# fnzhan/EMLight

Measured on AMD Instinct MI355X. Metric: training images/sec (regression step: DenseNet-BC fwd + Sinkhorn loss + bwd + Adam), higher is better.
Workload: dtype f32; 1 GPU; RegressionNetwork train step, BASELINE configs[1]; per_gpu_batch=64, global_batch=64, anchors=128, parallelism=single

## Files before the change

emlight_amd/RegressionNetwork/dense_engine_bwd.py:

```python
import ctypes
import os

import torch

from .. import _lib
from .._knobs import knob_choice, knob_flag


def _r16(v):
    return (v + 15) // 16 * 16


class _BwdBuffers:
    def gf12(self, r):
        if self.GF12[r] is None:
            self.GF12[r] = self._gf12_new()
        return self.GF12[r]

    def __init__(self, enc, ws, dev):
        f32 = dict(dtype=torch.float32, device=dev)
        self.G = [torch.zeros(blk["P"], blk["ld"], **f32) for blk in ws.blocks]
        self.GF = torch.zeros(ws.F.shape[0], ws.F.shape[1], **f32)
        maxP = ws.blocks[0]["P"]
        self.DZ = torch.empty(2, maxP, 48, **f32)
        self.ring = max(1, int(os.environ.get("EML_WGRAD_RING", 4))) if enc.overlap_wgrad(dev) else 1
        self.GF12 = [None] * self.ring
        self._gf12_new = lambda: torch.empty(maxP, 12, **f32)
        self.N12 = torch.empty(maxP, 12, **f32)
        self.TOP = torch.empty(2 * maxP * 12, **f32)
        kp, ko, g = enc.kp_max, max(enc.ko_max, 48), enc.grid_max
        self.Wd = [[torch.empty(lay["Kp"] * 48, **f32) for lay in blk["layers"]] for blk in ws.blocks]
        self.WdT = [torch.empty(blk["trans"]["Kp"] * blk["trans"]["Ko"], **f32) for blk in ws.blocks]
        self.permutes = None
        self.coef = torch.zeros(8, max(kp, ko), **f32)
        self.part2 = torch.zeros(2, g * kp * 2, dtype=torch.float64, device=dev)
        self.partW = torch.empty(g * max(kp * 48, 2 * 27 * 256, 4 * 1024), **f32)
        i32 = dict(dtype=torch.int32, device=dev)
        self.cond = [[torch.zeros(lay["Kp"], **i32) for lay in blk["layers"]] for blk in ws.blocks]
        self.condT = [torch.zeros(blk["trans"]["Kp"], **i32) for blk in ws.blocks]
        self.any_ill = torch.zeros(1, **i32)
        self.dg_grid = 128
        self.dg_scratch = torch.empty(self.dg_grid * kp, dtype=torch.float64, device=dev)
        self.side = None
        if enc.overlap_wgrad(dev):
            self.side = torch.cuda.Stream(device=dev)
            self.partW3 = [torch.empty(g * 2 * 27 * 256, **f32) for _ in range(self.ring)]
            self.ev_ready = [torch.cuda.Event() for _ in range(self.ring)]
            self.ev_done = [None] * self.ring


def run_backward(enc, ws, x, gpooled, need_x=False, need_params=None):
    if getattr(ws, "bwd", None) is None:
        ws.bwd = _BwdBuffers(enc, ws, x.device)
    L, p, st = _lib.lib(), _lib.ptr, _lib.current_stream()
    m = enc.model
    f = m.features
    if not m.training:
        raise NotImplementedError("HIP DenseNet backward is implemented for train-mode BatchNorm "
# ... 23 lines not shown
        for l_, lay_ in enumerate(blk_["layers"]):
            items.append((getattr(mod_, "denselayer%d" % (l_ + 1)).conv1.weight, bw.Wd[bi_][l_], 2, 48, lay_["Cin"],
                          lay_["Kp"], 48))
        tr_ = blk_["trans"]
        items.append((getattr(f, "transition%d" % (bi_ + 1)).conv.weight, bw.WdT[bi_], 2, tr_["Cout"], blk_["Ctot"],
                      tr_["Kp"], tr_["Ko"]))
    bw.permutes.launch(L, st, items)
    params = enc.param_list()
    if need_params is None:
        need_params = [True] * len(params)
    from .._dist import grad_slot
    grads = {}
    for q, need in zip(params, need_params):
        slot = grad_slot(q) if need else None
        grads[id(q)] = slot if slot is not None else torch.empty_like(q)
    gr = lambda q: p(grads[id(q)])
    coefs = [tuple(bw.coef[3 * k + i] for i in range(3)) for k in range(2)]
    cA, cB, cC = coefs[0]
    sB, sC = bw.coef[6], bw.coef[7]

    direct = knob_choice("EML_DGAMMA_DIRECT", "always", ("always", "never")) != "never"
    c3_fold = knob_flag("EML_C3_FOLD", True)
    c3_gf = knob_flag("EML_C3_GF", False)
    bw.any_ill.zero_()

    def dgamma_direct(blk, X_ld, Pin, Hin, Win, pool, DY, ld_dy, Zr, ld_z, co, Cout, conv, Cin, scale1, shift1, cond, bn):
        if not direct:
            return
        a, b, c = co if co is not None else (None, None, None)
        _lib.check(L.eml_dense_bn_dgamma_direct_f32(
            p(blk["X"]), X_ld, Pin, Hin, Win, pool, p(DY), ld_dy, p(Zr), ld_z, p(a), p(b), p(c), Cout, p(conv.weight), Cin,
            p(scale1), p(shift1), p(blk["mean"]), p(blk["istd"]), p(cond), p(bw.dg_scratch), gr(bn.weight), bw.dg_grid, st),
            "eml_dense_bn_dgamma_direct_f32")

    def finalize(R, pstride, count, bn, mean, istd, C, Cpad, coef=0, s_acc=None, src=None, c_lo=0, c_hi=None, conv=None,
                 cond=None):
        a, b, c = coefs[coef] if coef is not None else (None, None, None)
        wargs = (p(bn.bias), p(conv.weight), gr(conv.weight), conv.weight.shape[0]) if conv is not None else (None, None, None, 0)
        _lib.check(L.eml_dense_bn_bwd_finalize_f32(
            p(part if src is None else src), R, pstride, float(count), p(bn.weight), p(mean), p(istd), C, Cpad, 1,
            gr(bn.weight), gr(bn.bias), p(a), p(b), p(c),
            p(sB) if s_acc is not None else None, p(sC) if s_acc is not None else None, int(bool(s_acc)),
            c_lo, Cpad if c_hi is None else c_hi, *wargs, p(cond), p(bw.any_ill) if cond is not None else None, st),
            "eml_dense_bn_bwd_finalize_f32")

    def parr(tensors):
# ... 52 lines not shown
                                          p(part), G3d, p(blk["X"]), ld, cin, p(sB), p(sC), p(bw.gf12(r)) if c3_gf else None,
                                          p(lay["scale2"]), p(lay["shift2"]), p(bw.partW), gr(Lm.conv2.weight), *drop, st), fn)
            else:
                fn = "eml_dense_conv3x3_bwd_data_drop_f32" if drop else "eml_dense_conv3x3_bwd_data_f32"
                _lib.check(getattr(L, fn)(*gsrc, p(Lm.conv2.weight), p(z), p(lay["zmean"]), p(lay["zistd"]), p(dz), B, Hb, Wb,
                                          p(part), G3d, p(blk["X"]), ld, cin, p(sB), p(sC), p(bw.gf12(r)), *drop, st), fn)
            if fold:
                pass
            elif bw.side is None:
                _lib.check(L.eml_dense_conv3x3_bwd_weight_f32(p(bw.gf12(r)), 12, 0, p(z), p(lay["scale2"]),
                                                              p(lay["shift2"]), B, Hb, Wb, p(bw.partW),
                                                              gr(Lm.conv2.weight), G3, st),
                           "eml_dense_conv3x3_bwd_weight_f32")
            else:
                bw.ev_ready[r].record(main)
                bw.side.wait_event(bw.ev_ready[r])
                _lib.check(L.eml_dense_conv3x3_bwd_weight_f32(p(bw.gf12(r)), 12, 0, p(z), p(lay["scale2"]),
                                                              p(lay["shift2"]), B, Hb, Wb, p(bw.partW3[r]),
                                                              gr(Lm.conv2.weight), G3s, st_side),
                           "eml_dense_conv3x3_bwd_weight_f32")
                if bw.ev_done[r] is None:
                    bw.ev_done[r] = torch.cuda.Event()
                bw.ev_done[r].record(bw.side)
            finalize(G3d, 96, P, Lm.norm2, lay["zmean"], lay["zistd"], 48, 48, coef=slot)
            a, b, c = coefs[slot]
            _lib.check(L.eml_dense_conv1x1_bwd_weight_f32(
                p(blk["X"]), ld, P, Hb, Wb, 0, kp, cin, p(lay["scale1"]), p(lay["shift1"]), p(dz), 48, p(z), 48,
                p(a), p(b), p(c), 48, p(bw.partW), gr(Lm.conv1.weight), Gw, p(dz),
                *((p(Lm.conv1.weight), narrow_lo, *((p(top2[0]), 12) if top else (p(Gbuf), ld)), p(bw.N12),
                   p(bw.part2[slot])) if narrow_lo is not None
                  else (None, 0, None, 0, None, None)), st), "eml_dense_conv1x1_bwd_weight_f32")
            return Lm

        def dgrad(layers, slots, k_lo, k_hi, top=False):
            lays = [blk["layers"][l] for l in layers]
            if top:
                _lib.check(L.eml_dense_conv1x1_bwd_data_multi_top_f32(
                    parr([bw.DZ[s_] for s_ in slots]), parr([bw.Wd[bi][l_] for l_ in layers]),
                    parr([y["scale1"] for y in lays]), parr([y["shift1"] for y in lays]),
                    parr([bw.part2[s_] for s_ in slots]), (ctypes.c_int * len(layers))(*[y["Kp"] for y in lays]),
                    P, k_hi, p(Gbuf), ld, Gd, parr([y["mask"] for y in lays]), p(top2), st),
                    "eml_dense_conv1x1_bwd_data_multi_top_f32")
                return
            _lib.check(L.eml_dense_conv1x1_bwd_data_multi_f32(
                len(layers), parr([bw.DZ[s_] for s_ in slots]), None, None, None, None,
                parr([bw.Wd[bi][l_] for l_ in layers]),
                parr([y["scale1"] for y in lays]), parr([y["shift1"] for y in lays]),
                parr([bw.part2[s_] for s_ in slots]), (ctypes.c_int * len(layers))(*[y["Kp"] for y in lays]),
                None, ld, None, None, P, k_lo, k_hi, p(Gbuf), ld, Gd,
                parr([y["mask"] for y in lays]), st),
                "eml_dense_conv1x1_bwd_data_multi_f32")

        def bn1_finalize(l, Lm, slot, c_lo, c_hi, rows=None):
            lay = blk["layers"][l]
            finalize(Gd if rows is None else rows, 2 * lay["Kp"], P, Lm.norm1, blk["mean"], blk["istd"], lay["Cin"], lay["Kp"], coef=None,
                     s_acc=True, src=bw.part2[slot], c_lo=c_lo, c_hi=c_hi, conv=Lm.conv1, cond=bw.cond[bi][l])

        def bn1_direct(l, Lm, slot):
            lay = blk["layers"][l]
            dgamma_direct(blk, ld, P, Hb, Wb, 0, bw.DZ[slot], 48, None, 0, None, 48, Lm.conv1, lay["Cin"], lay["scale1"],
                          lay["shift1"], bw.cond[bi][l], Lm.norm1)

        l = len(blk["layers"]) - 1
        have_top = False
        while l >= 0:
            if l >= 1:
                la, lb = l, l - 1
                cin_a, cin_b = blk["layers"][la]["Cin"], blk["layers"][lb]["Cin"]
                Lma = conv2_backward(la, 0, narrow_lo=cin_b, top=have_top)
                bn1_finalize(la, Lma, 0, cin_b, cin_a, rows=Gw)
                Lmb = conv2_backward(lb, 1, n12=True)
                to_top = (lb >= 2 and blk["layers"][la]["mask"] is not None and bw.side is None
                          and cin_b >= 24 and cin_b % 4 == 0)
                dgrad([la, lb], [0, 1], 0, cin_b, top=to_top)
                have_top = to_top
                bn1_finalize(la, Lma, 0, 0, cin_b)
                bn1_finalize(lb, Lmb, 1, 0, blk["layers"][lb]["Kp"])
                bn1_direct(la, Lma, 0)
                bn1_direct(lb, Lmb, 1)
                l -= 2
            else:
                Lm0 = conv2_backward(l, 0)
                dgrad([l], [0], 0, blk["layers"][l]["Cin"])
                bn1_finalize(l, Lm0, 0, 0, blk["layers"][l]["Kp"])
                bn1_direct(l, Lm0, 0)
                l -= 1
        c0b = blk["C0"]
        norm0_fused = bi == 0 and knob_flag("EML_NORM0_FUSED", True) and c0b % 4 == 0 and c0b <= 32
        if not norm0_fused:
            materialize(Gbuf, blk, 0, c0b)
        dY, ld_dy = Gbuf, ld
    b0 = ws.blocks[0]
    c0 = enc.c_init
    if norm0_fused:
        _lib.check(L.eml_dense_norm0_bwd_stats_f32(p(dY), ld_dy, p(ws.Y0), c0, p(ws.scale0), p(ws.shift0), p(sB), p(sC), c0,
                                                   b0["P"], p(ws.mean0), p(ws.istd0), p(part), Gb, st),
                   "eml_dense_norm0_bwd_stats_f32")
    else:
        _lib.check(L.eml_dense_bn_bwd_stats_f32(p(dY), ld_dy, p(ws.Y0), c0, p(b0["X"]), b0["ld"], 1, c0, b0["P"],
                                                p(ws.mean0), p(ws.istd0), p(part), Gb, st), "eml_dense_bn_bwd_stats_f32")
    finalize(Gb, 2 * c0, b0["P"], f.norm0, ws.mean0, ws.istd0, c0, _r16(c0), coef=0)
    if norm0_fused:
# ... 18 lines not shown
```

emlight_amd/_knobs.py:

```python
import os
import sys

_seen = {}


def _note(name, value, default):
    if value != default:
        print("emlight_amd: A/B knob %s=%r (default %r)" % (name, value, default), file=sys.stderr)


def knob_int(name, default, lo=None, hi=None):
    raw = os.environ.get(name)
    if ("int", name, raw) not in _seen:
        val = default
        if raw is not None:
            try:
                val = int(raw)
                if (lo is not None and val < lo) or (hi is not None and val > hi):
                    raise ValueError("out of range")
            except ValueError:
                print("emlight_amd: ignoring %s=%r (want an integer%s); using %r"
                      % (name, raw, "" if lo is None else " >= %d" % lo, default), file=sys.stderr)
                val = default
        _note(name, val, default)
# ... 8 lines not shown
        if raw is not None:
            if raw in ("0", "1"):
                val = raw == "1"
            else:
                print("emlight_amd: ignoring %s=%r (want 0 or 1); using %d" % (name, raw, int(default)), file=sys.stderr)
        _note(name, val, bool(default))
        _seen[("flag", name, raw)] = val
    return _seen[("flag", name, raw)]


def knob_choice(name, default, choices):
    raw = os.environ.get(name)
    if ("choice", name, raw) not in _seen:
        val = default
        if raw is not None:
            if raw in choices:
                val = raw
            else:
                print("emlight_amd: ignoring %s=%r (want one of %s); using %r" % (name, raw, "/".join(choices), default),
                      file=sys.stderr)
        _note(name, val, default)
        _seen[("choice", name, raw)] = val
    return _seen[("choice", name, raw)]
```

emlight_amd/_lib.py:

```python
import ctypes
import os
import threading

_HERE = os.path.dirname(os.path.abspath(__file__))
LIB_PATH = os.environ.get("EML_LIB_PATH") or os.path.join(_HERE, "libemlight_hip.so")

_f32p = ctypes.c_void_p
_i32p = ctypes.c_void_p
_f64p = ctypes.c_void_p
_stream = ctypes.c_void_p
_int = ctypes.c_int
_u64 = ctypes.c_ulonglong

ABI_VERSION = 31

SIGNATURES = {
    "eml_abi_version": (_int, []),
    "eml_last_error": (ctypes.c_char_p, []),
    "eml_sg_rasterise_f32": (_int, [_f32p, _f32p, _f32p, _f32p, _int, _int, _int, _int, _stream]),
    "eml_sg_rasterise_ex_f32": (_int, [_f32p, _f32p, _f32p, _f32p, _int, _int, _int, _int, _int, ctypes.c_void_p, _stream]),
    "eml_sg_rasterise_bwd_colors_f32": (_int, [_f32p, _f32p, _f32p, _f32p, _int, _int, _int, _int, _stream]),
    "eml_emd_anchor_cost_f32": (_int, [_f32p, _f32p, _int, _stream]),
    "eml_sinkhorn_schedule_f32": (_int, [_f32p, _f32p, ctypes.c_long, ctypes.c_double, ctypes.c_double, _int,
                                         ctypes.c_double, _f32p, _f32p, _i32p, _f32p, _stream]),
# ... 202 lines not shown
    "eml_sphere_render_bwd_work_floats": (ctypes.c_size_t, [_int, _int, _int, _int]),
    "eml_sphere_render_bwd_f32": (_int, [_f32p, _int, _int, _int, _int, ctypes.c_double, _int, ctypes.c_double, _i32p, _i32p,
                                         _f32p, _f32p, _f32p, _stream]),
    "eml_sphere_mirror_taps_f32": (_int, [_int, _int, _int, ctypes.c_double, _i32p, _f32p, _stream]),
    "eml_gm_anchor_cost_f32": (_int, [ctypes.c_void_p, _int, _int, _int, _f32p, _f32p, _stream]),
    "eml_sinkhorn_fwd_cost_f32": (_int, [_f32p, _f32p, _f32p, _f32p, _f32p, _f32p, ctypes.c_double, ctypes.c_double, _int,
                                         ctypes.c_double, _f32p, _f32p, _i32p, _f32p, _f32p, _f32p, _f32p, _f32p, _int, _int,
                                         _int, _int, ctypes.c_double, _f32p, ctypes.c_long, _stream]),
    "eml_sphere_max_pool_fwd_f32": (_int, [_f32p, _i32p, _f32p, _f32p, ctypes.c_void_p, _int, _int, _int, _int, _stream]),
    "eml_sphere_max_pool_bwd_f32": (_int, [_f32p, ctypes.c_void_p, _i32p, _i32p, _f32p, _f32p, _int, _int, _int, _int, _stream]),
    "eml_sphere_conv_small_dbias_f32": (_int, [_f32p, _f32p, ctypes.c_float, _f32p, _f32p, _int, _int, _int, _int, _stream]),
    "eml_env_prefilter_work_floats": (ctypes.c_size_t, [_int, _int, _int, _int, _int]),
    "eml_env_prefilter_f32": (_int, [_f32p, _int, _int, _int, _int, _int, ctypes.c_void_p, _f32p, _f32p, _stream]),
    "eml_gbuffer_shade_f32": (_int, [_f32p, _int, _f32p, _int, ctypes.c_long, _f32p, _int, ctypes.c_long, _f32p, _f32p, _f32p,
                                     _f32p, _f32p, _int, _int, _int, ctypes.c_double, ctypes.c_double, _f32p, _f32p, _f32p,
                                     ctypes.c_double, _f32p, _stream]),
    "eml_env_prefilter_bwd_work_floats": (ctypes.c_size_t, [_int, _int, _int, _int, _int]),
    "eml_env_prefilter_bwd_f32": (_int, [_f32p, _int, _int, _int, _int, _int, ctypes.c_void_p, _f32p, _f32p, _stream]),
    "eml_gbuffer_shade_bwd_work_floats": (ctypes.c_size_t, [_int, _int, _int, _int, _int, _int, _int, _int, _int]),
    "eml_gbuffer_shade_bwd_f32": (_int, [_f32p, _f32p, _int, _f32p, _int, ctypes.c_long, _f32p, _int, ctypes.c_long, _f32p,
                                         _f32p, _f32p, _f32p, _f32p, _int, _int, _int, ctypes.c_double, ctypes.c_double,
                                         _f32p, _f32p, ctypes.c_double, _f32p, _f32p, _f32p, _f32p, _f32p, _f32p, _f32p,
                                         _f32p, _stream]),
}

_lock = threading.Lock()
_lib = None


class EmlightHipError(RuntimeError):
    pass


def lib():
    global _lib
    if _lib is not None:
        return _lib
    with _lock:
        if _lib is not None:
            return _lib
        if not os.path.exists(LIB_PATH):
            raise EmlightHipError(
                "libemlight_hip.so not found at %s -- build it with "
                "`python -c 'import __graft_entry__ as g; g.build()'` or `make -C emlight_amd/csrc`. "
                "There is no CPU fallback." % LIB_PATH)
        handle = ctypes.CDLL(LIB_PATH)
# ... 52 lines not shown
```

emlight_amd/csrc/dense_bwd.hip:

```cpp
#include "eml_common.h"
#include "eml_dropout.h"

#include <cstdint>
#include <cstdlib>
#include <type_traits>

namespace {

using eml::f32x4;
using eml::f4c;
using eml::mfma16;
using eml::shfl_xor_d;

constexpr int kTH = 8, kTW = 32, kHH = kTH + 2, kHW = kTW + 2;

constexpr int kPSG = 14;
constexpr int kBD = 512;
constexpr int kGRows = 2;
constexpr int kGPass = kHH / kGRows;

template <bool FUSE, bool WIDE, bool DROP = false>
__global__ __launch_bounds__(kBD, 2) void conv3x3_bwd_data_kernel(
    const float* __restrict__ G, int ldg, int c0, const float* __restrict__ W2, const float* __restrict__ Z,
    const float* __restrict__ zmean, const float* __restrict__ zistd, float* __restrict__ DZ, int B, int H, int W,
// ... 1543 lines not shown
    }
  }
  __syncthreads();
  for (int e = tid; e < Kp * 2; e += 256)
    partials[(size_t)blockIdx.x * Kp * 2 + e] =
        (sacc[e] + sacc[(size_t)Kp * 2 + e]) + (sacc[(size_t)2 * Kp * 2 + e] + sacc[(size_t)3 * Kp * 2 + e]);
}

struct BwdLayer {
  const float* DZ;
  const float* Zr;
  const float* cA;
  const float* cB;
  const float* cC;
  const float* Wd;
  const float* scale1;
  const float* shift1;
  double* partials;
  int Kp;
};

template <int NL, int MT , bool RAW = false ,
          bool MASKED = false, bool TOP = false>
__global__ __launch_bounds__(256, 2) void conv1x1_bwd_data_multi_kernel(BwdLayer L0, BwdLayer L1,
                                                                        const float* __restrict__ X, int ldx,
                                                                        const float* __restrict__ mean,
                                                                        const float* __restrict__ istd, int P,
                                                                        int k_lo, int k_hi, float* __restrict__ Gd,
                                                                        int ldg, int KpMax,
                                                                        const unsigned long long* __restrict__ M0,
                                                                        const unsigned long long* __restrict__ M1,
                                                                        float* __restrict__ Top) {
  extern __shared__ __attribute__((aligned(16))) float smem[];
  double* sacc = reinterpret_cast<double*>(smem);
  float* vec_l = reinterpret_cast<float*>(sacc + (size_t)NL * 4 * KpMax * 2);
  const int tid = threadIdx.x, lane = tid & 63, wave = tid >> 6;
  const int r = lane & 15, kk = lane >> 4;
  const BwdLayer Ls[2] = {L0, L1};
  for (int e = tid; e < NL * 4 * KpMax * 2; e += 256) sacc[e] = 0.0;
  for (int e = tid; e < KpMax; e += 256) {
    vec_l[e] = MASKED ? 0.f : mean[e];
    vec_l[KpMax + e] = MASKED ? 0.f : istd[e];
#pragma unroll
    for (int j = 0; j < NL; ++j) {
      vec_l[(2 + 2 * j) * KpMax + e] = e < Ls[j].Kp ? Ls[j].scale1[e] : 0.f;
      vec_l[(3 + 2 * j) * KpMax + e] = e < Ls[j].Kp ? Ls[j].shift1[e] : 0.f;
    }
  }
  __syncthreads();
  constexpr int TP = 64 * MT;
  const int ntiles = (P + TP - 1) / TP;
  const int nt_lo = k_lo >> 4, nt_hi = (k_hi + 15) >> 4;
  constexpr int NCH = 2;

  float4 wq[2][3][NCH];
  auto load_w = [&](int j, int nt0, float4 (&dst)[3][NCH]) {
    const int nnt = Ls[j].Kp >> 4;
#pragma unroll
    for (int jo = 0; jo < 3; ++jo)
#pragma unroll
      for (int n = 0; n < NCH; ++n) {
        const int nt = min(nt0 + n, nnt - 1);
// ... 37 lines not shown
            dz[j][jo][m].z = fmaf(a4.z, dy.z, fmaf(b4.z, zr.z, c4.z));
            dz[j][jo][m].w = fmaf(a4.w, dy.w, fmaf(b4.w, zr.w, c4.w));
          }
        }
      }
    for (int nt0 = nt_lo; nt0 < nt_hi; nt0 += NCH) {
      float4 gs[MT][NCH], xv[MT][NCH];
#pragma unroll
      for (int n = 0; n < NCH; ++n) {
        const int k4 = 16 * min(nt0 + n, nt_hi - 1) + 4 * kk;
        const int k4l = (k4 + 3 >= k_lo && k4 < k_hi) ? k4 : (k_lo & ~3);
#pragma unroll
        for (int m = 0; m < MT; ++m) {
          gs[m][n] = *reinterpret_cast<const float4*>(Gd + prow[m] * ldg + k4l);
          if constexpr (!MASKED) xv[m][n] = *reinterpret_cast<const float4*>(X + prow[m] * ldx + k4l);
        }
      }
      const int nt_next = nt0 + NCH < nt_hi ? nt0 + NCH : nt_lo;
#pragma unroll
      for (int j = 0; j < NL; ++j) {
        const int nnt = Ls[j].Kp >> 4;
        unsigned long long mk[MT][NCH][4];
        if constexpr (MASKED) {
          const unsigned long long* __restrict__ Mj = j == 0 ? M0 : M1;
#pragma unroll
          for (int m = 0; m < MT; ++m)
#pragma unroll
            for (int n = 0; n < NCH; ++n) {
              const size_t wi =
                  ((size_t)__builtin_amdgcn_readfirstlane((p0 >> 4) + m) * nnt + min(nt0 + n, nnt - 1)) * 4;
#pragma unroll
              for (int g = 0; g < 4; ++g) mk[m][n][g] = Mj[wi + g];
            }
        }
        const int cur = NL == 2 ? j : wsel;
        if (j + 1 < NL)
          load_w(j + 1, nt0, wq[cur ^ 1]);
        else
          load_w(0, nt_next, wq[cur ^ 1]);
        __builtin_amdgcn_sched_barrier(0);
        f32x4 acc[MT][NCH];
#pragma unroll
        for (int m = 0; m < MT; ++m)
#pragma unroll
          for (int n = 0; n < NCH; ++n) acc[m][n] = f32x4{0.f, 0.f, 0.f, 0.f};
#pragma unroll
        for (int jo = 0; jo < 3; ++jo)
#pragma unroll
          for (int t = 0; t < 4; ++t)
#pragma unroll
            for (int n = 0; n < NCH; ++n)
#pragma unroll
              for (int m = 0; m < MT; ++m) acc[m][n] = mfma16(f4c(wq[cur][jo][n], t), f4c(dz[j][jo][m], t), acc[m][n]);
        if (NL == 1) wsel ^= 1;
        double* my = sacc + ((size_t)(j * 4 + wave) * KpMax) * 2;
#pragma unroll
        for (int n = 0; n < NCH; ++n) {
          const int nt = nt0 + n;
          if (nt < nnt && nt < nt_hi) {
            const int k4 = 16 * nt + 4 * kk;
            const float4 mu = *reinterpret_cast<const float4*>(vec_l + k4);
            const float4 is = *reinterpret_cast<const float4*>(vec_l + KpMax + k4);
            const float4 sk = *reinterpret_cast<const float4*>(vec_l + (2 + 2 * j) * KpMax + k4);
            const float4 tk = *reinterpret_cast<const float4*>(vec_l + (3 + 2 * j) * KpMax + k4);
            const bool in0 = k4 + 0 >= k_lo && k4 + 0 < k_hi, in1 = k4 + 1 >= k_lo && k4 + 1 < k_hi;
            const bool in2 = k4 + 2 >= k_lo && k4 + 2 < k_hi, in3 = k4 + 3 >= k_lo && k4 + 3 < k_hi;
            unsigned long long inb[4] = {0ull, 0ull, 0ull, 0ull};
            if constexpr (MASKED) {
              inb[0] = __ballot(in0);
              inb[1] = __ballot(in1);
              inb[2] = __ballot(in2);
              inb[3] = __ballot(in3);
            }
            float l1[4] = {0.f, 0.f, 0.f, 0.f}, l2[4] = {0.f, 0.f, 0.f, 0.f};
#pragma unroll
            for (int m = 0; m < MT; ++m) {
              float d0, d1, d2, d3;
              if constexpr (MASKED) {
// ... 6 lines not shown
                d0 = (pv[m] && in0 && fmaf(x.x, sk.x, tk.x) > 0.f) ? acc[m][n][0] : 0.f;
                d1 = (pv[m] && in1 && fmaf(x.y, sk.y, tk.y) > 0.f) ? acc[m][n][1] : 0.f;
                d2 = (pv[m] && in2 && fmaf(x.z, sk.z, tk.z) > 0.f) ? acc[m][n][2] : 0.f;
                d3 = (pv[m] && in3 && fmaf(x.w, sk.w, tk.w) > 0.f) ? acc[m][n][3] : 0.f;
                l2[0] = fmaf(d0, (x.x - mu.x) * is.x, l2[0]);
                l2[1] = fmaf(d1, (x.y - mu.y) * is.y, l2[1]);
                l2[2] = fmaf(d2, (x.z - mu.z) * is.z, l2[2]);
                l2[3] = fmaf(d3, (x.w - mu.w) * is.w, l2[3]);
              }
              gs[m][n].x = fmaf(sk.x, d0, gs[m][n].x);
              gs[m][n].y = fmaf(sk.y, d1, gs[m][n].y);
              gs[m][n].z = fmaf(sk.z, d2, gs[m][n].z);
              gs[m][n].w = fmaf(sk.w, d3, gs[m][n].w);
              l1[0] += d0;
              l1[1] += d1;
              l1[2] += d2;
              l1[3] += d3;
            }
#pragma unroll
            for (int g = 0; g < 4; ++g) {
              l1[g] = eml::row16_sum(l1[g]);
              if constexpr (!MASKED) l2[g] = eml::row16_sum(l2[g]);
              if (r == 0) {
                my[2 * (k4 + g)] += (double)l1[g];
                if constexpr (!MASKED) my[2 * (k4 + g) + 1] += (double)l2[g];
              }
            }
          }
        }
      }
#pragma unroll
      for (int n = 0; n < NCH; ++n) {
        const int nt = nt0 + n;
        if (nt < nt_hi) {
          const int k4 = 16 * nt + 4 * kk;
          const bool act = k4 + 3 >= k_lo && k4 < k_hi;
          if constexpr (TOP) {
            const int t = k4 - (k_hi - 24);
            float* cdst = Top + (t >= 12 ? (size_t)P * 12 + (t - 12) : (size_t)max(t, 0));
#pragma unroll
            for (int m = 0; m < MT; ++m) {
              float* dst = t >= 0 ? cdst + prow[m] * 12 : Gd + prow[m] * ldg + k4;
              if (pv[m] && act) *reinterpret_cast<float4*>(dst) = gs[m][n];
            }
          } else {
#pragma unroll
            for (int m = 0; m < MT; ++m) {
              if (pv[m] && act) *reinterpret_cast<float4*>(Gd + prow[m] * ldg + k4) = gs[m][n];
            }
          }
        }
      }
    }
  }
  __syncthreads();
#pragma unroll
  for (int j = 0; j < NL; ++j) {
    const int Kp = Ls[j].Kp;
    const double* base = sacc + (size_t)j * 4 * KpMax * 2;
    for (int e = tid; e < Kp * 2; e += 256)
      Ls[j].partials[(size_t)blockIdx.x * Kp * 2 + e] = (base[e] + base[(size_t)KpMax * 2 + e]) +
                                                        (base[(size_t)2 * KpMax * 2 + e] + base[(size_t)3 * KpMax * 2 + e]);
  }
}

template <int MT>
__global__ __launch_bounds__(256, 2) void conv1x1_bwd_narrow_kernel(
    const float* __restrict__ DZ, const float* __restrict__ W1 , int Cin, int k_lo,
    const float* __restrict__ X, int ldx, const float* __restrict__ scale1, const float* __restrict__ shift1,
    const float* __restrict__ mean, const float* __restrict__ istd, int P, const float* __restrict__ Gd, int ldg,
    float* __restrict__ N12, double* __restrict__ partials , int Kp) {
  __shared__ double red[4][12][2];
  const int tid = threadIdx.x, lane = tid & 63, wave = tid >> 6;
  const int r = lane & 15, kk = lane >> 4;
  float aw[3][4];
#pragma unroll
  for (int jo = 0; jo < 3; ++jo)
#pragma unroll
    for (int t = 0; t < 4; ++t) aw[jo][t] = r < 12 ? W1[(size_t)(16 * jo + 4 * kk + t) * Cin + k_lo + r] : 0.f;
  const bool cv = kk < 3;
  const int cq = k_lo + 4 * (cv ? kk : 2);
  float sk[4], tk[4], mu[4], is[4];
#pragma unroll
  for (int g = 0; g < 4; ++g) {
    sk[g] = scale1[cq + g];
// ... 844 lines not shown
      else if (relu_mask16 && !accumulate && Ko == 160) EML_LAUNCH_TRANSITION_RES(10);
      else if (relu_mask16 && !accumulate && Ko == 176) EML_LAUNCH_TRANSITION_RES(11);
      else if (relu_mask16) {
        if (accumulate) EML_LAUNCH_TRANSITION(true, true); else EML_LAUNCH_TRANSITION(false, true);
      } else {
        if (accumulate) EML_LAUNCH_TRANSITION(true, false); else EML_LAUNCH_TRANSITION(false, false);
      }
#undef EML_LAUNCH_TRANSITION
#undef EML_LAUNCH_TRANSITION_RES
    }
  } else {
    if (Ko == 48) EML_LAUNCH_BWD_DATA(false, true, 2); else EML_LAUNCH_BWD_DATA(false, false, 4);
  }
#undef EML_LAUNCH_BWD_DATA
  return eml::check_launch("eml_dense_conv1x1_bwd_data_f32");
}

namespace {
int launch_bwd_data_multi(int n_layers, const float* const* DZ, const float* const* Zr, const float* const* cA,
                          const float* const* cB, const float* const* cC, const float* const* Wd,
                          const float* const* scale1, const float* const* shift1, double* const* partials, const int* Kp,
                          const float* X, int ldx, const float* mean, const float* istd, long P, int k_lo, int k_hi,
                          float* G, int ldg, int grid, const unsigned long long* const* relu_masks, float* top,
                          eml_stream_t stream) {
  if (top && (n_layers != 2 || !relu_masks || Zr || k_lo != 0 || k_hi < 24 || (k_hi & 3) || P * 12 > 2147483647L))
    return eml::fail(EML_EINVAL, "eml_dense_conv1x1_bwd_data_multi_top_f32: the compact top-24 output needs two layers, "
                                 "relu_masks, materialised dz, k_lo == 0 and k_hi >= 24, a multiple of 4 (k_hi=%d)", k_hi);
  if (n_layers < 1 || n_layers > 2 || !DZ || !Wd || !scale1 || !shift1 || !partials ||
      !Kp || (!relu_masks && (!X || !mean || !istd)) || !G || P < 1 || grid < 1 || k_lo < 0 || k_hi <= k_lo ||
      (ldx & 3) || (ldg & 3))
    return eml::fail(EML_EINVAL, "eml_dense_conv1x1_bwd_data_multi_f32: bad arguments");
  const bool raw = Zr == nullptr;
  if (!raw && (!cA || !cB || !cC))
    return eml::fail(EML_EINVAL, "eml_dense_conv1x1_bwd_data_multi_f32: Zr given without cA/cB/cC");
  if (relu_masks && !raw)
    return eml::fail(EML_EINVAL, "eml_dense_conv1x1_bwd_data_multi_f32: relu_masks needs the materialised dz (Zr == NULL)");
  BwdLayer L[2];
  const unsigned long long* Mk[2] = {nullptr, nullptr};
  int kmax = 0;
  for (int j = 0; j < 2; ++j) {
    const int s = j < n_layers ? j : 0;
    const unsigned long long* mk = relu_masks ? relu_masks[s] : nullptr;
    Mk[j] = mk;
    L[j] = raw ? BwdLayer{DZ[s], nullptr, nullptr, nullptr, nullptr, Wd[s], scale1[s], shift1[s], partials[s], Kp[s]}
               : BwdLayer{DZ[s], Zr[s], cA[s], cB[s], cC[s], Wd[s], scale1[s], shift1[s], partials[s], Kp[s]};
    if (!DZ[s] || (!raw && !Zr[s]) || !Wd[s] || !partials[s] || (relu_masks && !mk) || (Kp[s] & 15) ||
        (!relu_masks && Kp[s] > ldx) || Kp[s] > ldg)
      return eml::fail(EML_EINVAL, "eml_dense_conv1x1_bwd_data_multi_f32: bad layer %d", s);
    if (Kp[s] > kmax) kmax = Kp[s];
  }
  if (((k_hi + 15) & ~15) > kmax) return eml::fail(EML_EINVAL, "eml_dense_conv1x1_bwd_data_multi_f32: range beyond Kp");
  const size_t lds = (size_t)n_layers * 4 * kmax * 2 * sizeof(double) + (size_t)(2 + 2 * n_layers) * kmax * sizeof(float);
  if (lds > 80 * 1024) return eml::fail(EML_EINVAL, "eml_dense_conv1x1_bwd_data_multi_f32: Kp=%d does not fit LDS", kmax);
#define EML_LAUNCH_MULTI(NLV, MTV, RAWV, MSKV)                                                                       \
  do {                                                                                                              \
    EML_ENSURE_LDS((&conv1x1_bwd_data_multi_kernel<NLV, MTV, RAWV, MSKV>), lds);                                 \
    hipLaunchKernelGGL((conv1x1_bwd_data_multi_kernel<NLV, MTV, RAWV, MSKV>), dim3(grid), dim3(256), lds,            \
                       (hipStream_t)stream, L[0], L[1], X, ldx, mean, istd, (int)P, k_lo, k_hi, G, ldg, kmax,        \
                       Mk[0], Mk[1], (float*)nullptr);                                                              \
  } while (0)
  if (n_layers == 1) {
    if (relu_masks) EML_LAUNCH_MULTI(1, 4, true, true);
    else if (raw) EML_LAUNCH_MULTI(1, 4, true, false);
    else EML_LAUNCH_MULTI(1, 4, false, false);
  } else if (top) {
    EML_ENSURE_LDS((&conv1x1_bwd_data_multi_kernel<2, 2, true, true, true>), lds);
    hipLaunchKernelGGL((conv1x1_bwd_data_multi_kernel<2, 2, true, true, true>), dim3(grid), dim3(256), lds,
                       (hipStream_t)stream, L[0], L[1], X, ldx, mean, istd, (int)P, k_lo, k_hi, G, ldg, kmax, Mk[0], Mk[1],
                       top);
  } else {
    if (relu_masks) EML_LAUNCH_MULTI(2, 2, true, true);
    else if (raw) EML_LAUNCH_MULTI(2, 2, true, false);
    else EML_LAUNCH_MULTI(2, 2, false, false);
  }
#undef EML_LAUNCH_MULTI
  return eml::check_launch("eml_dense_conv1x1_bwd_data_multi_f32");
}
}

extern "C" int eml_dense_conv1x1_bwd_data_multi_f32(int n_layers, const float* const* DZ, const float* const* Zr,
                                                    const float* const* cA, const float* const* cB,
                                                    const float* const* cC, const float* const* Wd,
                                                    const float* const* scale1, const float* const* shift1,
                                                    double* const* partials, const int* Kp, const float* X, int ldx,
                                                    const float* mean, const float* istd, long P, int k_lo, int k_hi,
                                                    float* G, int ldg, int grid,
                                                    const unsigned long long* const* relu_masks, eml_stream_t stream) {
  return launch_bwd_data_multi(n_layers, DZ, Zr, cA, cB, cC, Wd, scale1, shift1, partials, Kp, X, ldx, mean, istd, P, k_lo,
                               k_hi, G, ldg, grid, relu_masks, nullptr, stream);
}

extern "C" int eml_dense_conv1x1_bwd_data_multi_top_f32(const float* const* DZ, const float* const* Wd,
                                                        const float* const* scale1, const float* const* shift1,
                                                        double* const* partials, const int* Kp, long P, int k_hi,
                                                        float* G, int ldg, int grid,
                                                        const unsigned long long* const* relu_masks, float* top,
                                                        eml_stream_t stream) {
  if (!top) return eml::fail(EML_EINVAL, "eml_dense_conv1x1_bwd_data_multi_top_f32: top is NULL");
  return launch_bwd_data_multi(2, DZ, nullptr, nullptr, nullptr, nullptr, Wd, scale1, shift1, partials, Kp, nullptr, 0,
                               nullptr, nullptr, P, 0, k_hi, G, ldg, grid, relu_masks, top, stream);
}

extern "C" int eml_dense_conv1x1_bwd_narrow_f32(const float* DZ, const float* W1, int Cin, int k_lo, const float* X,
                                                int ldx, const float* scale1, const float* shift1, const float* mean,
                                                const float* istd, long P, const float* G, int ldg, float* N12,
                                                double* partials, int Kp, int grid, eml_stream_t stream) {
  if (!DZ || !W1 || !X || !scale1 || !shift1 || !mean || !istd || !G || !N12 || !partials || P < 1 || grid < 1 ||
      k_lo < 0 || (k_lo & 1) || k_lo + 12 > Cin || Cin > Kp || (ldx & 1) || (ldg & 1) || Kp > ldx || Kp > ldg)
    return eml::fail(EML_EINVAL, "eml_dense_conv1x1_bwd_narrow_f32: bad arguments");
  hipLaunchKernelGGL((conv1x1_bwd_narrow_kernel<4>), dim3(grid), dim3(256), 0, (hipStream_t)stream, DZ, W1, Cin, k_lo, X,
                     ldx, scale1, shift1, mean, istd, (int)P, G, ldg, N12, partials, Kp);
  return eml::check_launch("eml_dense_conv1x1_bwd_narrow_f32");
}

extern "C" int eml_dense_grad_materialize_f32(float* G, int ldg, const float* X, int ldx, const float* sB,
                                              const float* sC, int c0, int n, long P, eml_stream_t stream) {
  if (!G || !X || !sB || !sC || P < 1 || n < 2 || (n & 1) || (c0 & 1) || (ldg & 1) || (ldx & 1))
    return eml::fail(EML_EINVAL, "eml_dense_grad_materialize_f32: bad arguments");
  const size_t total = (size_t)P * (n >> 1);
  const int grid = (int)((total + 255) / 256 < 8192 ? (total + 255) / 256 : 8192);
  hipLaunchKernelGGL(grad_materialize_kernel, dim3(grid), dim3(256), 0, (hipStream_t)stream, G, ldg, X, ldx, sB, sC, c0,
                     n, (size_t)P);
  return eml::check_launch("eml_dense_grad_materialize_f32");
}
// ... 99 lines not shown
```

include/emlight_hip_ext.h:

```cpp
#ifndef EMLIGHT_HIP_EXT_H
#define EMLIGHT_HIP_EXT_H

#include "emlight_hip.h"

#ifdef __cplusplus
extern "C" {
#endif

int eml_pano_warp_f32(const float* pano, int B, int H, int W, int h, int w, double theta_deg, double phi_deg, double move,
                      const double* params_dev, float* out, double* coords, eml_stream_t stream);

size_t eml_pano_warp_bwd_work_floats(int B, int H, int W, int h, int w, int want_dpano, int want_dparams);
int eml_pano_warp_bwd_f32(const float* grad_out, const float* pano, int B, int H, int W, int h, int w, double theta_deg,
                          double phi_deg, double move, const double* params_dev, float* dpano, double* dparams, float* work,
                          eml_stream_t stream);

size_t eml_sphere_render_bwd_work_floats(int B, int H, int W, int S);
int eml_sphere_render_bwd_f32(const float* grad_out, int B, int H, int W, int S, double view_azimuth_deg, int materials_mask,
                              double phong_m, const int* mirror_csr_ptr, const int* mirror_csr_src, const float* mirror_csr_w,
                              float* dpano, float* work, eml_stream_t stream);

int eml_sphere_mirror_taps_f32(int H, int W, int S, double view_azimuth_deg, int* idx, float* wgt, eml_stream_t stream);

int eml_gm_anchor_cost_f32(const void* depth, int depth_is_f64, int B, int N, float* anchors_out, float* M_out,
// ... 17 lines not shown
size_t eml_env_prefilter_work_floats(int B, int H, int W, int Ho, int L);
int eml_env_prefilter_f32(const float* pano, int B, int H, int W, int Ho, int L, const double* lobes, float* out, float* work,
                          eml_stream_t stream);

int eml_gbuffer_shade_f32(const float* pano, int H, const float* e_diffuse, int Hd, long d_stride, const float* e_phong, int Hg,
                          long g_stride, const float* normal, const float* coverage, const float* kd, const float* ks,
                          const float* km, int B, int h, int w, double fov_deg, double view_azimuth_deg, float* shaded,
                          const float* background, const float* exposure, double gamma, float* composite,
                          eml_stream_t stream);

size_t eml_env_prefilter_bwd_work_floats(int B, int H, int W, int Ho, int L);
int eml_env_prefilter_bwd_f32(const float* grad_out, int B, int H, int W, int Ho, int L, const double* lobes, float* dpano,
                              float* work, eml_stream_t stream);

size_t eml_gbuffer_shade_bwd_work_floats(int B, int H, int Hd, int Hg, int h, int w, int want_dpano, int want_d_e_diffuse,
                                         int want_d_e_phong);
int eml_gbuffer_shade_bwd_f32(const float* grad_out, const float* pano, int H, const float* e_diffuse, int Hd, long d_stride,
                              const float* e_phong, int Hg, long g_stride, const float* normal, const float* coverage,
                              const float* kd, const float* ks, const float* km, int B, int h, int w, double fov_deg,
                              double view_azimuth_deg, const float* shaded, const float* exposure, double gamma, float* dkd,
                              float* dks, float* dkm, float* d_e_diffuse, float* d_e_phong, float* dpano, float* dshaded,
                              float* work, eml_stream_t stream);

#ifdef __cplusplus
}
#endif

#endif
```

Baseline: 575.5 images/s.

## Add optional four-layer fused conv1x1 data-grad pass and trim masked kernel LDS

Adds an extended conv1x1 backward-data entry point that can process four dense layers in one launch. Two layer pairs are handled together, with a 24-channel top slice computed early and the rest deferred, which cuts launches and re-reads of the gradient buffer. The kernel also halves its shared-memory accumulator in the masked variant, which only needs one double per channel, and skips redundant MFMAs on the last partial output tile. The four-layer path is gated behind EML_DGRAD_QUAD_KMIN, which defaults to all zeros, so by default only the LDS trim and edge-tile change take effect.

```diff
diff --git a/emlight_amd/RegressionNetwork/dense_engine_bwd.py b/emlight_amd/RegressionNetwork/dense_engine_bwd.py
--- a/emlight_amd/RegressionNetwork/dense_engine_bwd.py
+++ b/emlight_amd/RegressionNetwork/dense_engine_bwd.py
@@ -4,7 +4,7 @@
 import torch
 
 from .. import _lib
-from .._knobs import knob_choice, knob_flag
+from .._knobs import knob_choice, knob_flag, knob_ints
 
 
 def _r16(v):
@@ -16,6 +16,10 @@
         if self.GF12[r] is None:
             self.GF12[r] = self._gf12_new()
         return self.GF12[r]
+
+    def slots(self, n):
+        if self.DZ.shape[0] < n:
+            self.DZ, self.part2 = self._dz_new(n), self._part2_new(n)
 
     def __init__(self, enc, ws, dev):
         f32 = dict(dtype=torch.float32, device=dev)
@@ -23,6 +27,7 @@
         self.GF = torch.zeros(ws.F.shape[0], ws.F.shape[1], **f32)
         maxP = ws.blocks[0]["P"]
         self.DZ = torch.empty(2, maxP, 48, **f32)
+        self._dz_new = lambda n: torch.empty(n, maxP, 48, **f32)
         self.ring = max(1, int(os.environ.get("EML_WGRAD_RING", 4))) if enc.overlap_wgrad(dev) else 1
         self.GF12 = [None] * self.ring
         self._gf12_new = lambda: torch.empty(maxP, 12, **f32)
@@ -34,6 +39,7 @@
         self.permutes = None
         self.coef = torch.zeros(8, max(kp, ko), **f32)
         self.part2 = torch.zeros(2, g * kp * 2, dtype=torch.float64, device=dev)
+        self._part2_new = lambda n: torch.zeros(n, g * kp * 2, dtype=torch.float64, device=dev)
         self.partW = torch.empty(g * max(kp * 48, 2 * 27 * 256, 4 * 1024), **f32)
         i32 = dict(dtype=torch.int32, device=dev)
         self.cond = [[torch.zeros(lay["Kp"], **i32) for lay in blk["layers"]] for blk in ws.blocks]
@@ -103,6 +109,12 @@
     direct = knob_choice("EML_DGAMMA_DIRECT", "always", ("always", "never")) != "never"
     c3_fold = knob_flag("EML_C3_FOLD", True)
     c3_gf = knob_flag("EML_C3_GF", False)
+    quad_q = getattr(L, "eml_dense_conv1x1_bwd_data_quad_supported", None)
+    quad = knob_flag("EML_DGRAD_QUAD", True) and bw.side is None and quad_q is not None and quad_q() == 1
+    quad_kmin = knob_ints("EML_DGRAD_QUAD_KMIN", (0, 0, 0))
+    quad = quad and any(quad_kmin)
+    if quad:
+        bw.slots(4)
     bw.any_ill.zero_()
 
     def dgamma_direct(blk, X_ld, Pin, Hin, Win, pool, DY, ld_dy, Zr, ld_z, co, Cout, conv, Cin, scale1, shift1, cond, bn):
@@ -201,8 +213,8 @@
                 if bw.ev_done[r] is None:
                     bw.ev_done[r] = torch.cuda.Event()
                 bw.ev_done[r].record(bw.side)
-            finalize(G3d, 96, P, Lm.norm2, lay["zmean"], lay["zistd"], 48, 48, coef=slot)
-            a, b, c = coefs[slot]
+            finalize(G3d, 96, P, Lm.norm2, lay["zmean"], lay["zistd"], 48, 48, coef=slot & 1)
+            a, b, c = coefs[slot & 1]
             _lib.check(L.eml_dense_conv1x1_bwd_weight_f32(
                 p(blk["X"]), ld, P, Hb, Wb, 0, kp, cin, p(lay["scale1"]), p(lay["shift1"]), p(dz), 48, p(z), 48,
                 p(a), p(b), p(c), 48, p(bw.partW), gr(Lm.conv1.weight), Gw, p(dz),
@@ -230,6 +242,15 @@
                 parr([y["mask"] for y in lays]), st),
                 "eml_dense_conv1x1_bwd_data_multi_f32")
 
+        def dgrad_ex(layers, slots, k_lo, k_hi, top=False):
+            lays = [blk["layers"][l] for l in layers]
+            _lib.check(L.eml_dense_conv1x1_bwd_data_multi_ex_f32(
+                len(layers), parr([bw.DZ[s_] for s_ in slots]), parr([bw.Wd[bi][l_] for l_ in layers]),
+                parr([y["scale1"] for y in lays]), parr([y["shift1"] for y in lays]),
+                parr([bw.part2[s_] for s_ in slots]), (ctypes.c_int * len(layers))(*[y["Kp"] for y in lays]),
+                P, k_lo, k_hi, p(Gbuf), ld, Gd, parr([y["mask"] for y in lays]), p(top2) if top else None, st),
+                "eml_dense_conv1x1_bwd_data_multi_ex_f32")
+
         def bn1_finalize(l, Lm, slot, c_lo, c_hi, rows=None):
             lay = blk["layers"][l]
             finalize(Gd if rows is None else rows, 2 * lay["Kp"], P, Lm.norm1, blk["mean"], blk["istd"], lay["Cin"], lay["Kp"], coef=None,
@@ -242,21 +263,45 @@
 
         l = len(blk["layers"]) - 1
         have_top = False
+        held = None
+        kmin = quad_kmin[min(bi, len(quad_kmin) - 1)]
         while l >= 0:
             if l >= 1:
                 la, lb = l, l - 1
+                s0 = 2 if held is not None else 0
                 cin_a, cin_b = blk["layers"][la]["Cin"], blk["layers"][lb]["Cin"]
-                Lma = conv2_backward(la, 0, narrow_lo=cin_b, top=have_top)
-                bn1_finalize(la, Lma, 0, cin_b, cin_a, rows=Gw)
-                Lmb = conv2_backward(lb, 1, n12=True)
-                to_top = (lb >= 2 and blk["layers"][la]["mask"] is not None and bw.side is None
-                          and cin_b >= 24 and cin_b % 4 == 0)
-                dgrad([la, lb], [0, 1], 0, cin_b, top=to_top)
-                have_top = to_top
-                bn1_finalize(la, Lma, 0, 0, cin_b)
-                bn1_finalize(lb, Lmb, 1, 0, blk["layers"][lb]["Kp"])
-                bn1_direct(la, Lma, 0)
-                bn1_direct(lb, Lmb, 1)
+                Lma = conv2_backward(la, s0, narrow_lo=cin_b, top=have_top)
+                bn1_finalize(la, Lma, s0, cin_b, cin_a, rows=Gw)
+                Lmb = conv2_backward(lb, s0 + 1, n12=True)
+                masked = blk["layers"][la]["mask"] is not None and bw.side is None
+                to_top = lb >= 2 and masked and cin_b >= 24 and cin_b % 4 == 0
+                kp_b = blk["layers"][lb]["Kp"]
+                if quad and kmin > 0 and masked and held is None and lb >= 2 and cin_b >= max(kmin, 24):
+                    dgrad_ex([la, lb], [0, 1], cin_b - 24, cin_b, top=to_top)
+                    have_top = to_top
+                    bn1_finalize(la, Lma, 0, cin_b - 24, cin_b)
+                    bn1_finalize(lb, Lmb, 1, cin_b - 24, kp_b)
+                    held = (la, lb, Lma, Lmb)
+                elif held is not None:
+                    ha, hb, Lmha, Lmhb = held
+                    dgrad_ex([ha, hb, la, lb], [0, 1, 2, 3], 0, cin_b, top=to_top)
+                    have_top = to_top
+                    bn1_finalize(ha, Lmha, 0, 0, cin_b)
+                    bn1_finalize(hb, Lmhb, 1, 0, cin_b)
+                    bn1_finalize(la, Lma, 2, 0, cin_b)
+                    bn1_finalize(lb, Lmb, 3, 0, kp_b)
+                    bn1_direct(ha, Lmha, 0)
+                    bn1_direct(hb, Lmhb, 1)
+                    bn1_direct(la, Lma, 2)
+                    bn1_direct(lb, Lmb, 3)
+                    held = None
+                else:
+                    dgrad([la, lb], [0, 1], 0, cin_b, top=to_top)
+                    have_top = to_top
+                    bn1_finalize(la, Lma, 0, 0, cin_b)
+                    bn1_finalize(lb, Lmb, 1, 0, kp_b)
+                    bn1_direct(la, Lma, 0)
+                    bn1_direct(lb, Lmb, 1)
                 l -= 2
             else:
                 Lm0 = conv2_backward(l, 0)
diff --git a/emlight_amd/_knobs.py b/emlight_amd/_knobs.py
--- a/emlight_amd/_knobs.py
+++ b/emlight_amd/_knobs.py
@@ -54,3 +54,21 @@
         _note(name, val, default)
         _seen[("choice", name, raw)] = val
     return _seen[("choice", name, raw)]
+
+
+def knob_ints(name, default):
+    raw = os.environ.get(name)
+    if ("ints", name, raw) not in _seen:
+        val = tuple(default)
+        if raw is not None:
+            try:
+                val = tuple(int(v) for v in raw.split(","))
+                if len(val) != len(default) or min(val) < 0:
+                    raise ValueError("wrong length or negative")
+            except ValueError:
+                print("emlight_amd: ignoring %s=%r (want %d integers >= 0, comma-separated); using %r"
+                      % (name, raw, len(default), tuple(default)), file=sys.stderr)
+                val = tuple(default)
+        _note(name, val, tuple(default))
+        _seen[("ints", name, raw)] = val
+    return _seen[("ints", name, raw)]
diff --git a/emlight_amd/_lib.py b/emlight_amd/_lib.py
--- a/emlight_amd/_lib.py
+++ b/emlight_amd/_lib.py
@@ -248,6 +248,9 @@
                                          _f32p, _f32p, _f32p, _f32p, _int, _int, _int, ctypes.c_double, ctypes.c_double,
                                          _f32p, _f32p, ctypes.c_double, _f32p, _f32p, _f32p, _f32p, _f32p, _f32p, _f32p,
                                          _f32p, _stream]),
+    "eml_dense_conv1x1_bwd_data_multi_ex_f32": (_int, [_int] + [ctypes.c_void_p] * 6 + [ctypes.c_long, _int, _int, _f32p, _int,
+                                                       _int, ctypes.c_void_p, _f32p, _stream]),
+    "eml_dense_conv1x1_bwd_data_quad_supported": (_int, []),
 }
 
 _lock = threading.Lock()
diff --git a/emlight_amd/csrc/dense_bwd.hip b/emlight_amd/csrc/dense_bwd.hip
--- a/emlight_amd/csrc/dense_bwd.hip
+++ b/emlight_amd/csrc/dense_bwd.hip
@@ -1589,22 +1589,25 @@
 
 template <int NL, int MT , bool RAW = false ,
           bool MASKED = false, bool TOP = false>
-__global__ __launch_bounds__(256, 2) void conv1x1_bwd_data_multi_kernel(BwdLayer L0, BwdLayer L1,
-                                                                        const float* __restrict__ X, int ldx,
+__global__ __launch_bounds__(256, 2) void conv1x1_bwd_data_multi_kernel(BwdLayer L0, BwdLayer L1, BwdLayer L2,
+                                                                        BwdLayer L3, const float* __restrict__ X, int ldx,
                                                                         const float* __restrict__ mean,
                                                                         const float* __restrict__ istd, int P,
                                                                         int k_lo, int k_hi, float* __restrict__ Gd,
                                                                         int ldg, int KpMax,
                                                                         const unsigned long long* __restrict__ M0,
                                                                         const unsigned long long* __restrict__ M1,
+                                                                        const unsigned long long* __restrict__ M2,
+                                                                        const unsigned long long* __restrict__ M3,
                                                                         float* __restrict__ Top) {
+  constexpr int SW = MASKED ? 1 : 2;
   extern __shared__ __attribute__((aligned(16))) float smem[];
   double* sacc = reinterpret_cast<double*>(smem);
-  float* vec_l = reinterpret_cast<float*>(sacc + (size_t)NL * 4 * KpMax * 2);
+  float* vec_l = reinterpret_cast<float*>(sacc + (size_t)NL * 4 * KpMax * SW);
   const int tid = threadIdx.x, lane = tid & 63, wave = tid >> 6;
   const int r = lane & 15, kk = lane >> 4;
-  const BwdLayer Ls[2] = {L0, L1};
-  for (int e = tid; e < NL * 4 * KpMax * 2; e += 256) sacc[e] = 0.0;
+  const BwdLayer Ls[4] = {L0, L1, L2, L3};
+  for (int e = tid; e < NL * 4 * KpMax * SW; e += 256) sacc[e] = 0.0;
   for (int e = tid; e < KpMax; e += 256) {
     vec_l[e] = MASKED ? 0.f : mean[e];
     vec_l[KpMax + e] = MASKED ? 0.f : istd[e];
@@ -1688,7 +1691,7 @@
         const int nnt = Ls[j].Kp >> 4;
         unsigned long long mk[MT][NCH][4];
         if constexpr (MASKED) {
-          const unsigned long long* __restrict__ Mj = j == 0 ? M0 : M1;
+          const unsigned long long* __restrict__ Mj = j == 0 ? M0 : j == 1 ? M1 : j == 2 ? M2 : M3;
 #pragma unroll
           for (int m = 0; m < MT; ++m)
 #pragma unroll
@@ -1699,7 +1702,7 @@
               for (int g = 0; g < 4; ++g) mk[m][n][g] = Mj[wi + g];
             }
         }
-        const int cur = NL == 2 ? j : wsel;
+        const int cur = NL % 2 == 0 ? (j & 1) : wsel;
         if (j + 1 < NL)
           load_w(j + 1, nt0, wq[cur ^ 1]);
         else
@@ -1710,16 +1713,25 @@
         for (int m = 0; m < MT; ++m)
 #pragma unroll
           for (int n = 0; n < NCH; ++n) acc[m][n] = f32x4{0.f, 0.f, 0.f, 0.f};
-#pragma unroll
-        for (int jo = 0; jo < 3; ++jo)
-#pragma unroll
-          for (int t = 0; t < 4; ++t)
-#pragma unroll
-            for (int n = 0; n < NCH; ++n)
-#pragma unroll
-              for (int m = 0; m < MT; ++m) acc[m][n] = mfma16(f4c(wq[cur][jo][n], t), f4c(dz[j][jo][m], t), acc[m][n]);
+        if (nt0 + 1 < nnt && nt0 + 1 < nt_hi) {
+#pragma unroll
+          for (int jo = 0; jo < 3; ++jo)
+#pragma unroll
+            for (int t = 0; t < 4; ++t)
+#pragma unroll
+              for (int n = 0; n < NCH; ++n)
+#pragma unroll
+                for (int m = 0; m < MT; ++m) acc[m][n] = mfma16(f4c(wq[cur][jo][n], t), f4c(dz[j][jo][m], t), acc[m][n]);
+        } else {
+#pragma unroll
+          for (int jo = 0; jo < 3; ++jo)
+#pragma unroll
+            for (int t = 0; t < 4; ++t)
+#pragma unroll
+              for (int m = 0; m < MT; ++m) acc[m][0] = mfma16(f4c(wq[cur][jo][0], t), f4c(dz[j][jo][m], t), acc[m][0]);
+        }
         if (NL == 1) wsel ^= 1;
-        double* my = sacc + ((size_t)(j * 4 + wave) * KpMax) * 2;
+        double* my = sacc + ((size_t)(j * 4 + wave) * KpMax) * SW;
 #pragma unroll
         for (int n = 0; n < NCH; ++n) {
           const int nt = nt0 + n;
@@ -1772,7 +1784,7 @@
               l1[g] = eml::row16_sum(l1[g]);
               if constexpr (!MASKED) l2[g] = eml::row16_sum(l2[g]);
               if (r == 0) {
-                my[2 * (k4 + g)] += (double)l1[g];
+                my[SW * (k4 + g)] += (double)l1[g];
                 if constexpr (!MASKED) my[2 * (k4 + g) + 1] += (double)l2[g];
               }
             }
@@ -1807,10 +1819,18 @@
 #pragma unroll
   for (int j = 0; j < NL; ++j) {
     const int Kp = Ls[j].Kp;
-    const double* base = sacc + (size_t)j * 4 * KpMax * 2;
-    for (int e = tid; e < Kp * 2; e += 256)
-      Ls[j].partials[(size_t)blockIdx.x * Kp * 2 + e] = (base[e] + base[(size_t)KpMax * 2 + e]) +
-                                                        (base[(size_t)2 * KpMax * 2 + e] + base[(size_t)3 * KpMax * 2 + e]);
+    const double* base = sacc + (size_t)j * 4 * KpMax * SW;
+    if constexpr (MASKED) {
+      for (int e = tid; e < Kp; e += 256) {
+        double* dst = Ls[j].partials + ((size_t)blockIdx.x * Kp + e) * 2;
+        dst[0] = (base[e] + base[(size_t)KpMax + e]) + (base[(size_t)2 * KpMax + e] + base[(size_t)3 * KpMax + e]);
+        dst[1] = 0.0;
+      }
+    } else {
+      for (int e = tid; e < Kp * 2; e += 256)
+        Ls[j].partials[(size_t)blockIdx.x * Kp * 2 + e] = (base[e] + base[(size_t)KpMax * 2 + e]) +
+                                                          (base[(size_t)2 * KpMax * 2 + e] + base[(size_t)3 * KpMax * 2 + e]);
+    }
   }
 }
 
@@ -2701,11 +2721,12 @@
                           const float* const* scale1, const float* const* shift1, double* const* partials, const int* Kp,
                           const float* X, int ldx, const float* mean, const float* istd, long P, int k_lo, int k_hi,
                           float* G, int ldg, int grid, const unsigned long long* const* relu_masks, float* top,
-                          eml_stream_t stream) {
-  if (top && (n_layers != 2 || !relu_masks || Zr || k_lo != 0 || k_hi < 24 || (k_hi & 3) || P * 12 > 2147483647L))
+                          eml_stream_t stream, bool ex = false) {
+  if (top && ((n_layers != 2 && !(ex && n_layers == 4)) || !relu_masks || Zr || (k_lo != 0 && !(ex && k_lo == k_hi - 24)) ||
+              k_hi < 24 || (k_hi & 3) || P * 12 > 2147483647L))
     return eml::fail(EML_EINVAL, "eml_dense_conv1x1_bwd_data_multi_top_f32: the compact top-24 output needs two layers, "
                                  "relu_masks, materialised dz, k_lo == 0 and k_hi >= 24, a multiple of 4 (k_hi=%d)", k_hi);
-  if (n_layers < 1 || n_layers > 2 || !DZ || !Wd || !scale1 || !shift1 || !partials ||
+  if (n_layers < 1 || (n_layers > 2 && !(ex && n_layers == 4)) || !DZ || !Wd || !scale1 || !shift1 || !partials ||
       !Kp || (!relu_masks && (!X || !mean || !istd)) || !G || P < 1 || grid < 1 || k_lo < 0 || k_hi <= k_lo ||
       (ldx & 3) || (ldg & 3))
     return eml::fail(EML_EINVAL, "eml_dense_conv1x1_bwd_data_multi_f32: bad arguments");
@@ -2714,10 +2735,10 @@
     return eml::fail(EML_EINVAL, "eml_dense_conv1x1_bwd_data_multi_f32: Zr given without cA/cB/cC");
   if (relu_masks && !raw)
     return eml::fail(EML_EINVAL, "eml_dense_conv1x1_bwd_data_multi_f32: relu_masks needs the materialised dz (Zr == NULL)");
-  BwdLayer L[2];
-  const unsigned long long* Mk[2] = {nullptr, nullptr};
+  BwdLayer L[4];
+  const unsigned long long* Mk[4] = {nullptr, nullptr, nullptr, nullptr};
   int kmax = 0;
-  for (int j = 0; j < 2; ++j) {
+  for (int j = 0; j < 4; ++j) {
     const int s = j < n_layers ? j : 0;
     const unsigned long long* mk = relu_masks ? relu_masks[s] : nullptr;
     Mk[j] = mk;
@@ -2729,30 +2750,34 @@
     if (Kp[s] > kmax) kmax = Kp[s];
   }
   if (((k_hi + 15) & ~15) > kmax) return eml::fail(EML_EINVAL, "eml_dense_conv1x1_bwd_data_multi_f32: range beyond Kp");
-  const size_t lds = (size_t)n_layers * 4 * kmax * 2 * sizeof(double) + (size_t)(2 + 2 * n_layers) * kmax * sizeof(float);
+  const size_t lds = (size_t)n_layers * 4 * kmax * (relu_masks ? 1 : 2) * sizeof(double) +
+                     (size_t)(2 + 2 * n_layers) * kmax * sizeof(float);
   if (lds > 80 * 1024) return eml::fail(EML_EINVAL, "eml_dense_conv1x1_bwd_data_multi_f32: Kp=%d does not fit LDS", kmax);
-#define EML_LAUNCH_MULTI(NLV, MTV, RAWV, MSKV)                                                                       \
+#define EML_LAUNCH_MULTI_TOP(NLV, MTV, RAWV, MSKV, TOPV, TOPP)                                                       \
   do {                                                                                                              \
-    EML_ENSURE_LDS((&conv1x1_bwd_data_multi_kernel<NLV, MTV, RAWV, MSKV>), lds);                                 \
-    hipLaunchKernelGGL((conv1x1_bwd_data_multi_kernel<NLV, MTV, RAWV, MSKV>), dim3(grid), dim3(256), lds,            \
-                       (hipStream_t)stream, L[0], L[1], X, ldx, mean, istd, (int)P, k_lo, k_hi, G, ldg, kmax,        \
-                       Mk[0], Mk[1], (float*)nullptr);                                                              \
+    EML_ENSURE_LDS((&conv1x1_bwd_data_multi_kernel<NLV, MTV, RAWV, MSKV, TOPV>), lds);                           \
+    hipLaunchKernelGGL((conv1x1_bwd_data_multi_kernel<NLV, MTV, RAWV, MSKV, TOPV>), dim3(grid), dim3(256), lds,      \
+                       (hipStream_t)stream, L[0], L[1], L[2], L[3], X, ldx, mean, istd, (int)P, k_lo, k_hi, G, ldg,   \
+                       kmax, Mk[0], Mk[1], Mk[2], Mk[3], TOPP);                                                     \
   } while (0)
+#define EML_LAUNCH_MULTI(NLV, MTV, RAWV, MSKV) EML_LAUNCH_MULTI_TOP(NLV, MTV, RAWV, MSKV, false, (float*)nullptr)
   if (n_layers == 1) {
     if (relu_masks) EML_LAUNCH_MULTI(1, 4, true, true);
     else if (raw) EML_LAUNCH_MULTI(1, 4, true, false);
     else EML_LAUNCH_MULTI(1, 4, false, false);
+  } else if (n_layers == 4) {
+    if (!relu_masks) return eml::fail(EML_EINVAL, "eml_dense_conv1x1_bwd_data_multi_ex_f32: four layers need relu_masks");
+    if (top) EML_LAUNCH_MULTI_TOP(4, 2, true, true, true, top);
+    else EML_LAUNCH_MULTI(4, 2, true, true);
   } else if (top) {
-    EML_ENSURE_LDS((&conv1x1_bwd_data_multi_kernel<2, 2, true, true, true>), lds);
-    hipLaunchKernelGGL((conv1x1_bwd_data_multi_kernel<2, 2, true, true, true>), dim3(grid), dim3(256), lds,
-                       (hipStream_t)stream, L[0], L[1], X, ldx, mean, istd, (int)P, k_lo, k_hi, G, ldg, kmax, Mk[0], Mk[1],
-                       top);
+    EML_LAUNCH_MULTI_TOP(2, 2, true, true, true, top);
   } else {
     if (relu_masks) EML_LAUNCH_MULTI(2, 2, true, true);
     else if (raw) EML_LAUNCH_MULTI(2, 2, true, false);
     else EML_LAUNCH_MULTI(2, 2, false, false);
   }
 #undef EML_LAUNCH_MULTI
+#undef EML_LAUNCH_MULTI_TOP
   return eml::check_launch("eml_dense_conv1x1_bwd_data_multi_f32");
 }
 }
@@ -2779,6 +2804,28 @@
   return launch_bwd_data_multi(2, DZ, nullptr, nullptr, nullptr, nullptr, Wd, scale1, shift1, partials, Kp, nullptr, 0,
                                nullptr, nullptr, P, 0, k_hi, G, ldg, grid, relu_masks, top, stream);
 }
+
+extern "C" int eml_dense_conv1x1_bwd_data_multi_ex_f32(int n_layers, const float* const* DZ, const float* const* Wd,
+                                                       const float* const* scale1, const float* const* shift1,
+                                                       double* const* partials, const int* Kp, long P, int k_lo,
+                                                       int k_hi, float* G, int ldg, int grid,
+                                                       const unsigned long long* const* relu_masks, float* top,
+                                                       eml_stream_t stream) {
+  if (n_layers != 1 && n_layers != 2 && n_layers != 4)
+    return eml::fail(EML_EINVAL, "eml_dense_conv1x1_bwd_data_multi_ex_f32: n_layers = %d (1, 2 or 4)", n_layers);
+  if (!DZ || !Wd || !scale1 || !shift1 || !partials || !Kp || !relu_masks)
+    return eml::fail(EML_EINVAL, "eml_dense_conv1x1_bwd_data_multi_ex_f32: NULL layer array (the pass is masked: relu_masks too)");
+  for (int j = 0; j < n_layers; ++j)
+    if (!DZ[j] || !Wd[j] || !scale1[j] || !shift1[j] || !partials[j] || !relu_masks[j])
+      return eml::fail(EML_EINVAL, "eml_dense_conv1x1_bwd_data_multi_ex_f32: NULL pointer in layer %d", j);
+  if (top && (n_layers == 1 || k_hi < 24 || (k_hi & 3) || (k_lo != 0 && k_lo != k_hi - 24)))
+    return eml::fail(EML_EINVAL, "eml_dense_conv1x1_bwd_data_multi_ex_f32: top needs 2 or 4 layers, k_hi >= 24, a multiple "
+                                 "of 4, and k_lo == 0 or k_hi - 24 (k_lo=%d, k_hi=%d)", k_lo, k_hi);
+  return launch_bwd_data_multi(n_layers, DZ, nullptr, nullptr, nullptr, nullptr, Wd, scale1, shift1, partials, Kp, nullptr, 0,
+                               nullptr, nullptr, P, k_lo, k_hi, G, ldg, grid, relu_masks, top, stream, true);
+}
+
+extern "C" int eml_dense_conv1x1_bwd_data_quad_supported(void) { return 1; }
 
 extern "C" int eml_dense_conv1x1_bwd_narrow_f32(const float* DZ, const float* W1, int Cin, int k_lo, const float* X,
                                                 int ldx, const float* scale1, const float* shift1, const float* mean,
diff --git a/include/emlight_hip_ext.h b/include/emlight_hip_ext.h
--- a/include/emlight_hip_ext.h
+++ b/include/emlight_hip_ext.h
@@ -63,6 +63,13 @@
                               float* dks, float* dkm, float* d_e_diffuse, float* d_e_phong, float* dpano, float* dshaded,
                               float* work, eml_stream_t stream);
 
+int eml_dense_conv1x1_bwd_data_multi_ex_f32(int n_layers, const float* const* DZ, const float* const* Wd,
+                                            const float* const* scale1, const float* const* shift1,
+                                            double* const* partials, const int* Kp, long P, int k_lo, int k_hi,
+                                            float* G, int ldg, int grid, const unsigned long long* const* relu_masks,
+                                            float* top, eml_stream_t stream);
+int eml_dense_conv1x1_bwd_data_quad_supported(void);
+
 #ifdef __cplusplus
 }
 #endif
```

Result: no change. 575.0 images/s (-0.1%).
